# kostastril/Aiyagari-Replication

Hardware: AMD Instinct MI355X
Metric: Bellman evals/sec (Na·Na'·Nz, fp64) (higher is better)
Workload: dtype f64; 1 GPU; aiyagari_vfi_sweep Na=20000 Nz=7 rouwenhorst (BASELINE configs[1]); Na=20000, Nz=7, search=exhaustive over a' (exact bound-tree screen)

## Files before the change

### aiyagari-replication_amd/csrc/bellman.hpp

```cpp
#pragma once
#include <hip/hip_runtime.h>
#include <stddef.h>

#include "dispatch.hpp"

namespace aiy {

struct BellArgs {
    int N, Na, Nl;
    bool keep_incoming;
    bool labor;
    int np;
    int coarse;
    int CK;
    int variant;
    double r, w, beta, sigma;
    const double* v_old;
    const double* a;
    const double* s;
    const double* P;
    const double* L;
    const double* dis;
    const int* hint;
    int* mom;
    const int* perm;
    int perm_slots;
    int tw;
    double* EV;
    double2* T;
    float* T32;
    double* Dm;
    double* Dt;
    double* Dm8;
    double* Dm512;
    int nb, nb8, nb512;
    bool tree;
    double* best0;
    int* idx0;
    int* kf;
    bool kf_valid;
    int* partial;
    int* touched;
    unsigned long long* hitcount;
    long long* trace;
// ... 120 lines not shown
```

### aiyagari-replication_amd/csrc/bellman_kernels.hip

```cpp
#include <hip/hip_ext.h>

#include <algorithm>
#include <type_traits>

#include "aiy_common.hpp"
#include "bell_dev.hpp"
#include "bellman.hpp"

namespace aiy {

__device__ __forceinline__ BellArgs bell_cand(const BellArgs& A, int c) {
    BellArgs B = A;
    const size_t o = (size_t)c * A.N * A.Na;
    B.r = A.rv[c];
    B.w = A.wv[c];
    B.v_old += o;
    B.EV += o;
    if (B.Dt) B.Dt += o;
    if (B.Dm8) B.Dm8 += (size_t)c * A.N * A.nb8;
    if (B.Dm512) B.Dm512 += (size_t)c * A.N * A.nb512;
    B.kf += o * A.Nl;
    B.best0 += o;
    B.idx0 += o;
    if (B.hint) B.hint += o;
// ... 735 lines not shown
                    int dir = kb >= hk + wnh ? 1 : (kb <= hk - wnh ? -1 : 0);
                    if (usem && kb >= hm - mw && kb <= hm + mw)
                        dir = kb == hm + mw ? 1 : (kb == hm - mw ? -1 : 0);
                    if (dir != 0 && !(A.variant & kVarNoClimb)) {
                        int k = kb, step = 2;
                        for (;;) {
                            const int kn = min(max(k + dir * step, 0), kf - 1);
                            if (kn == k || !take(kn)) break;
                            k = kn;
                            step <<= 1;
                        }
                        for (int s2 = step >> 1; s2 >= 1; s2 >>= 1) {
                            const int c0 = idx[r] / Nl;
                            if (c0 + s2 < kf) take(c0 + s2);
                            if (c0 - s2 >= 0) take(c0 - s2);
                        }
                    }
                }
            }
        } else {
            best[r] = A.best0[t];
            idx[r] = A.idx0[t] == -2 ? -1 : A.idx0[t];
        }
    }
    int q_su[R];
    double kp_su[R];
#pragma unroll
    for (int r = 0; r < R; ++r) {
        q_su[r] = idx[r];
        kp_su[r] = a[idx[r] >= 0 ? idx[r] / Nl : 0];
    }
    unsigned nhits = nsu, nsup = 0, nwv = 0, nblk = 0, ngt = 0, nfine = 0, lane_pairs = 0;
    unsigned npath[2] = {0, 0};
    const long long t_start = (INS && A.trace) ? (long long)wall_clock64() : 0;
    long long cyc[4] = {0, 0, 0, 0}, c_mark = (INS && A.trace) ? (long long)__builtin_amdgcn_s_memtime() : 0;
    const long long c_mark0 = c_mark;
    auto stamp = [&](int ph) __attribute__((always_inline)) {
        if (INS && A.trace) {
            const long long now = (long long)__builtin_amdgcn_s_memtime();
            cyc[ph] += now - c_mark;
            c_mark = now;
        }
    };
    stamp(0);

    auto exchange = [&]() __attribute__((always_inline)) {
        if constexpr (W > 1) {
#pragma unroll
            for (int r = 0; r < R; ++r)
                s_cand[lw][r * 64 + lane] = make_double2(best[r], (double)idx[r]);
            __syncthreads();
            for (int v = 0; v < W; ++v)
#pragma unroll
                for (int r = 0; r < R; ++r) {
                    const double2 e = s_cand[v][r * 64 + lane];
                    if (v != wave && (int)e.y >= 0) lexi_take(e.x, (int)e.y, best[r], idx[r]);
                }
            __syncthreads();
        }
    };

    for (int l0 = 0; l0 < Nl; l0 += LB) {
        double coh[R][LB], B[R][LB], dis[LB];
        int kg = 0;
        int kfl = 0x7fffffff;
#pragma unroll
// ... 161 lines not shown
#pragma unroll
            for (int kk = 0; kk < 8; ++kk)
                vote |= (__any(GF ? pk[kk] && kk < nk : pk[kk]) ? 1u : 0u) << kk;
            if constexpr (!GF) vote &= (1u << (k1 - k0)) - 1u;
            if (!vote) return;
            stamp(2);
            while (vote) {
                const int kk = __builtin_ctz(vote);
                vote &= vote - 1;
                const int k = k0 + kk;
                const double2 tkk = s_cand[lw][k - sbase];
#pragma unroll
                for (int r = 0; r < R; ++r)
#pragma unroll
                    for (int q = 0; q < LB; ++q) {
                        const double c = coh[r][q] - tkk.x;
                        const int lin = (l0 + q) + Nl * k;
                        if (lin != idx[r] && c > 0 && (!GF || kk < nk) &&
                            (tkk.y - B[r][q]) * aiy_ipow(c, NP) >= kThr) {
                            ++nhits;
                            const double val =
                                bell_val<NP, LAB>(c, ev[k], A.sigma, dis[q]);
                            if (lexi_take(val, lin, best[r], idx[r])) {
#pragma unroll
                                for (int q2 = 0; q2 < LB; ++q2)
                                    if (B[r][q2] == B[r][q2])
                                        B[r][q2] = screen_B(best[r], idx[r], dis[q2], NP);
                            }
                        }
                    }
            }
            stamp(3);
        };
        auto load8 = [&](int sb, double& dm8, double& a8) __attribute__((always_inline)) {
            const int sub = (sb << 6) + lane;
            const bool oku = sub < A.nb8;
            dm8 = oku ? A.Dm8[(size_t)i * A.nb8 + sub] : -__builtin_inf();
            a8 = oku ? a[sub << 3] : 0.0;
        };
        auto stage = [&](int sbase, unsigned long long pass, double2 (&st)[8])
                         __attribute__((always_inline)) {
            if constexpr (LEAN) {
                unsigned bm = 0;
#pragma unroll
                for (int b = 0; b < 8; ++b) bm |= ((pass >> (8 * b)) & 0xffull) ? 1u << b : 0u;
                while (bm) {
                    const int b0 = __builtin_ctz(bm);
                    bm &= bm - 1;
                    const int b1 = bm ? __builtin_ctz(bm) : -1;
                    if (bm) bm &= bm - 1;
                    const int k0 = min(sbase + (b0 << 6) + lane, Na - 1);
                    const double2 v0 = make_double2(a[k0], Drow[k0]);
                    double2 v1 = make_double2(0.0, 0.0);
                    if (b1 >= 0) {
                        const int k1 = min(sbase + (b1 << 6) + lane, Na - 1);
                        v1 = make_double2(a[k1], Drow[k1]);
                    }
                    s_cand[lw][(b0 << 6) + lane] = v0;
                    if (b1 >= 0) s_cand[lw][(b1 << 6) + lane] = v1;
                }
            } else {
#pragma unroll
                for (int b = 0; b < 8; ++b)
                    if ((pass >> (8 * b)) & 0xffull) {
                        const int k = min(sbase + (b << 6) + lane, Na - 1);
                        st[b] = make_double2(a[k], Drow[k]);
                    }
            }
        };
        auto prep = [&](int sb, int bsel, int bstep, double dm8, double a8, double2 (&st)[8],
                        unsigned long long& gmo, bool subsplit = false)
                        __attribute__((always_inline)) -> unsigned long long {
            stamp(0);
            const int sbase = sb << 9;
            if constexpr (GRP) {
                constexpr int NG = 64 / GL, CH = LEAN ? 4 : 8;
                static_assert(NG % CH == 0, "whole chunks of groups");
                unsigned long long any = 0;
#pragma unroll
                for (int g0 = 0; g0 < NG; g0 += CH) {
                    double cx[CH], dd[CH], t[CH];
#pragma unroll
                    for (int u = 0; u < CH; ++u) {
                        cx[u] = readlane_d(gC, (g0 + u) * GL) - a8;
                        dd[u] = dm8 - readlane_d(gB, (g0 + u) * GL);
                    }
                    AIY_SCHED_BARRIER();
                    screen_t<NP, CH>(t, cx, dd);
#pragma unroll
                    for (int u = 0; u < CH; ++u) any |= __ballot(t[u] >= kThr);
                }
                if (INS && (A.hitcount || A.trace)) ngt += NG;
                const int nfe = min(64, (kg - sbase + 7) >> 3);
                unsigned long long pass = any & (nfe >= 64 ? ~0ull : (1ull << nfe) - 1ull);
                if (bstep > 1) {
                    const unsigned long long one = subsplit ? 0x01ull : 0xffull;
                    unsigned long long pat = one << (subsplit ? bsel : 8 * bsel);
                    for (int sh = subsplit ? bstep : 8 * bstep; sh < 64; sh <<= 1) pat |= pat << sh;
                    pass &= pat;
                }
                if (INS && (A.hitcount || A.trace)) nblk += __builtin_popcountll(pass);
                unsigned long long keep = 0, own = 0;
                for (unsigned long long m = pass; m; m &= m - 1) {
                    const int u = __builtin_ctzll(m);
                    const double dv = readlane_d(dm8, u), av = readlane_d(a8, u);
                    double cx[RL], dd[RL], t[RL];
#pragma unroll
                    for (int r = 0; r < R; ++r)
#pragma unroll
                        for (int q = 0; q < LB; ++q) {
                            cx[r * LB + q] = coh[r][q] - av;
                            dd[r * LB + q] = dv - B[r][q];
                        }
                    screen_t<NP, RL>(t, cx, dd);
                    bool p = false;
#pragma unroll
                    for (int m2 = 0; m2 < RL; ++m2) p = p || t[m2] >= kThr;
                    if (__any(p)) keep |= 1ull << u;
                    if constexpr (GF) own |= p ? 1ull << u : 0ull;
                }
                pass = keep;
                if constexpr (GF) gmo = keep ? group_or_u64(own) : 0ull;
                if (INS && A.trace && lane == 0) lane_pairs += __builtin_popcountll(pass);
                stage(sbase, pass, st);
                stamp(1);
// ... 5 lines not shown
            dm64 = fmax(dm64, dpp_d<0x104>(dm64));
            const int nblock = min(8, (kg - sbase + 63) >> 6);
            unsigned own = 0;
            for (int b = subsplit ? 0 : bsel; b < nblock; b += subsplit ? 1 : bstep) own |= 1u << b;
            if (INS && (A.hitcount || A.trace)) nblk += __builtin_popcount(own);
            const unsigned bpass = mask8(dm64, a8, 0, 8, nblock) & own;
            unsigned long long pass = 0;
            const bool deal = subsplit && bstep > 1;
            int ord = 0;
            for (unsigned bm = bpass; bm; bm &= bm - 1, ++ord) {
                if (deal && ord % bstep != bsel) continue;
                const int b = __builtin_ctz(bm);
                const int nsub = min(8, (kg - (sbase + (b << 6)) + 7) >> 3);
                if (INS && (A.hitcount || A.trace)) nblk += nsub;
                pass |= (unsigned long long)mask8(dm8, a8, 8 * b, 1, nsub, true) << (8 * b);
            }
            if constexpr (W > 1) {
                if (deal) {
                    s_pass[bsel] = pass;
                    __syncthreads();
                    unsigned long long all = 0;
                    for (int v = 0; v < bstep; ++v) all |= s_pass[v];
                    __syncthreads();
                    const unsigned long long pat = bstep == 2 ? 0x5555555555555555ull
                                                 : (bstep == 4 ? 0x1111111111111111ull
                                                               : 0x0101010101010101ull);
                    pass = all & (pat << bsel);
                }
            }
            stage(sbase, pass, st);
            stamp(1);
            return pass;
        };
        auto finish = [&](int sb, unsigned long long pass, const double2 (&st)[8],
                          unsigned long long gm) __attribute__((always_inline)) {
            const int sbase = sb << 9;
            if constexpr (!LEAN)
#pragma unroll
                for (int b = 0; b < 8; ++b)
                    if ((pass >> (8 * b)) & 0xffull) s_cand[lw][(b << 6) + lane] = st[b];
            __builtin_amdgcn_wave_barrier();
            __builtin_amdgcn_fence(__ATOMIC_RELEASE, "wavefront");
            stamp(1);
            double2 tkA[8], tkB[8];
            unsigned long long pm = pass;
            if constexpr (LEAN) {
                for (; pm; pm &= pm - 1) {
                    const int b0 = __builtin_ctzll(pm);
                    load_tk(b0, tkA);
                    fine(sbase, sbase + (b0 << 3), min(sbase + (b0 << 3) + 8, kg), tkA);
                }
            }
            if constexpr (GF) {
                pm = 0;
                const int hb = 63 - __builtin_clzll(pass);
                const bool ncl = FAST && sbase + (hb << 3) + 8 <= kfmin;
                auto next = [&](int& k0) __attribute__((always_inline)) {
                    const unsigned lo = (unsigned)gm, hi = (unsigned)(gm >> 32);
                    const unsigned tl = lo ? (unsigned)__builtin_ctz(lo) : ~0u;
                    const unsigned th = hi ? ((unsigned)__builtin_ctz(hi) | 32u) : ~0u;
                    const int b = (int)min(min(tl, th), (unsigned)hb);
                    gm &= gm - 1;
                    k0 = sbase + (b << 3);
                    return b;
                };
                int kA, kB;
                bool actA = gm != 0, actB;
                load_tk(next(kA), tkA);
                for (;;) {
// ... 5 lines not shown
                    actA = gm != 0;
                    const bool moreA = __any(actA);
                    if (moreA) load_tk(next(kA), tkA);
                    fine(sbase, kB, 0, tkB, actB, ncl);
                    if (!moreA) break;
                }
            }
            if (pm) load_tk(__builtin_ctzll(pm), tkA);
            while (pm) {
                const int b0 = __builtin_ctzll(pm);
                pm &= pm - 1;
                if (pm) load_tk(__builtin_ctzll(pm), tkB);
                fine(sbase, sbase + (b0 << 3), min(sbase + (b0 << 3) + 8, kg), tkA);
                if (!pm) break;
                const int b1 = __builtin_ctzll(pm);
                pm &= pm - 1;
                if (pm) load_tk(__builtin_ctzll(pm), tkA);
                fine(sbase, sbase + (b1 << 3), min(sbase + (b1 << 3) + 8, kg), tkB);
            }
            stamp(2);
            __builtin_amdgcn_wave_barrier();
        };

        const int nsb = (kg + 511) >> 9;
        int sfirst = -1;
        {
            int hk = -1;
#pragma unroll
            for (int r = 0; r < R; ++r)
                if (idx[r] >= 0) hk = idx[r] / Nl;
            const unsigned long long m = __ballot(hk >= 0);
            if (m) sfirst = min(readlane_i(hk, __builtin_ctzll(m)) >> 9, nsb - 1);
        }
        double2 st_cur[8], st_prev[8];
        if (sfirst >= 0) {
            if (INS) ++nsup;
            double d8, a8;
            load8(sfirst, d8, a8);
            unsigned long long gm1 = 0;
            const unsigned long long p = prep(sfirst, wave, W, d8, a8, st_cur, gm1,
                                              (A.variant & kVarDealBlocks) != 0);
            if (p) finish(sfirst, p, st_cur, gm1);
            exchange();
            set_B();
        }
        double dm0, a0;
        auto load512 = [&](int g) __attribute__((always_inline)) {
            const int sbl = g + lane;
            const bool oks = sbl < nsb;
            dm0 = oks ? A.Dm512[(size_t)i * A.nb512 + sbl] : -__builtin_inf();
            a0 = oks ? a[sbl << 9] : 0.0;
        };
        if (l0 == 0) {
            dm0 = dm0_pre;
            a0 = a0_pre;
        } else {
            load512(0);
        }
        double bmin, cmax;
        {
            if constexpr (GRP) {
                if (sfirst >= 0) set_G();
                bmin = wave_rest_fmin_d(gB);
                cmax = wave_rest_fmax_d(gC);
            } else {
                double bl = __builtin_nan(""), cl = -__builtin_inf();
#pragma unroll
                for (int r = 0; r < R; ++r)
#pragma unroll
                    for (int q = 0; q < LB; ++q) {
                        bl = fmin(bl, B[r][q]);
                        cl = fmax(cl, (okr[r] && l0 + q < Nl) ? coh[r][q] : -__builtin_inf());
                    }
                bmin = wave_fmin_d(bl);
                cmax = wave_fmax_d(cl);
            }
        }
        int g = 0;
        unsigned long long sm = 0;
        auto test512 = [&]() __attribute__((always_inline)) {
            if (INS) ++nwv;
            unsigned long long m =
                __ballot(lane < nsb - g && screen_wave<NP>(dm0, a0, bmin, cmax));
            static_assert(64 % W == 0, "superblock g + u belongs to wave u % W");
            if constexpr (W > 1) m &= (~0ull / ((1ull << W) - 1ull)) << wave;
            if (sfirst >= g && sfirst < g + 64) m &= ~(1ull << (sfirst - g));
            return m;
        };
        if (nsb > 0) sm = test512();
        auto next_sb = [&]() __attribute__((always_inline)) -> int {
            for (;;) {
                if (sm) {
                    const int u = __builtin_ctzll(sm);
                    sm &= sm - 1;
                    if (INS) ++nsup;
                    return g + u;
                }
                g += 64;
                if (g >= nsb) return -1;
                load512(g);
                sm = test512();
            }
        };
        int cur = nsb > 0 ? next_sb() : -1;
        double pd = 0.0, pa = 0.0;
        if (cur >= 0) load8(cur, pd, pa);
        unsigned long long pass_prev = 0, gm_cur = 0, gm_prev = 0;
        int sb_prev = -1;
        while (cur >= 0) {
            const double d8 = pd, a8 = pa;
            const int nxt = next_sb();
            if (nxt >= 0) load8(nxt, pd, pa);
            const unsigned long long pc = prep(cur, 0, 1, d8, a8, st_cur, gm_cur);
            if constexpr (LEAN) {
                if (pc) finish(cur, pc, st_cur, gm_cur);
                cur = nxt;
                continue;
            }
            if (pass_prev) finish(sb_prev, pass_prev, st_prev, gm_prev);
#pragma unroll
            for (int b = 0; b < 8; ++b) st_prev[b] = st_cur[b];
            pass_prev = pc;
            gm_prev = gm_cur;
            sb_prev = cur;
            cur = nxt;
        }
        if (pass_prev) finish(sb_prev, pass_prev, st_prev, gm_prev);
    }

    exchange();
    const long long c_end = (INS && A.trace) ? (long long)__builtin_amdgcn_s_memtime() : 0;

    bool okd = false;
    double dmax = 0.0;
#pragma unroll
    for (int r = 0; r < R; ++r) {
        if (!okr[r] || wave != 0) continue;
        const size_t t = (size_t)i * Na + jbase + r * 64 + lane;
        double b = best[r];
        int q = idx[r];
        const double vo = vo_pre[r];
        if (!feas[r] && LAB) {
            b = A.keep_incoming ? A.v_new[t] : vo;
        } else {
            if (q < 0) {
                q = 0;
                b = __builtin_nan("");
            }
            const int l = q % Nl, k = q / Nl;
            double kp = kp_su[r];
            if (__ballot(q != q_su[r]) != 0ull) kp = a[k];
            A.idx[t] = q;
            if (A.pk) A.pk[t] = kp;
            if (A.pc) A.pc[t] = cash<LAB>(x[r], y, LAB ? A.L[l] : 1.0) - kp;
            if (LAB && A.pl) A.pl[t] = A.L[l];
        }
        A.v_new[t] = b;
        if (mom && A.hint) {
            const int sh = (hk0[r] >= 0 && idx[r] >= 0) ? idx[r] / Nl - hk0[r] : 0;
            const int shc = max(-32767, min(32767, sh));
// ... 27 lines not shown
            for (int c = 0; c < 4; ++c) {
                unsigned sum = 0;
                for (int v = 0; v < W; ++v) sum += s_cnt[v][c];
                sums[c] = sum;
            }
        }
        if (W == 1 ? lane == 0 : threadIdx.x == 0) {
            long long* tr = A.trace + 16 * (size_t)item;
            tr[0] = t_start;
            tr[1] = (long long)wall_clock64();
            tr[2] = (long long)(unsigned)__builtin_amdgcn_s_getreg((20 << 0) | (0 << 6) | (3 << 11)) |
                    ((long long)(unsigned)__builtin_amdgcn_s_getreg((4 << 0) | (0 << 6) | (31 << 11))
                     << 32);
            for (int c = 0; c < 4; ++c) tr[3 + c] = sums[c];
            tr[7] = block_id;
            for (int c = 0; c < 4; ++c) tr[8 + c] = cyc[c];
            tr[12] = t_boot;
            tr[13] = c_mark0 - c_boot;
            tr[14] = (long long)__builtin_amdgcn_s_memtime() - c_end;
            tr[15] = pairs;
        }
    }
    if (INS && A.hitcount) {
        unsigned long long* hc = A.hitcount + 4 * (blockIdx.x % kDiffSlots);
        if (nhits) atomicAdd(hc, (unsigned long long)nhits);
        if (lane == 0) {
            const unsigned long long ns = 64ull * R * LB;
            atomicAdd(hc + 1, nwv * 64ull);
            atomicAdd(hc + 2, nblk * ns + ngt * 64ull);
            if (nfine) atomicAdd(hc + 3, nfine * ns);
#pragma unroll
            for (int q = 0; q < 2; ++q)
                if (npath[q]) atomicAdd(hc + kPathBase + q, (unsigned long long)npath[q]);
        }
    }
}

template <int NP, bool LAB, int R, int LB, int W, bool INS, int PK, int WM>
__global__ __launch_bounds__(64 * W * PK, 3) void bell_tree_kernel(BellArgs A0, int ntile) {
    __shared__ double2 s_cand[W * PK][512];
    __shared__ unsigned long long s_pass[W];
    const int lw = PK > 1 ? readfirst(threadIdx.x >> 6) : 0;
    bell_tree_item<NP, LAB, R, LB, W, INS, PK, false, WM>(A0, ntile, (int)blockIdx.x * PK + lw,
                                                          (int)gridDim.x * PK, s_cand, s_pass);
}

template <int NP, bool INS>
__global__ __launch_bounds__(128, 3) void bell_tree_hybrid_kernel(BellArgs A0, int ntile) {
    __shared__ double2 s_cand[2][512];
    __shared__ unsigned long long s_pass[2];
    const int b = (int)blockIdx.x;
    if (A0.perm[2 * b + 1] == -2) {
        bell_tree_item<NP, false, 1, 1, 2, INS, 1, true>(A0, ntile, 2 * b, 2 * (int)gridDim.x,
                                                        s_cand, s_pass);
    } else {
        const int lw = readfirst(threadIdx.x >> 6);
        bell_tree_item<NP, false, 1, 1, 1, INS, 2, true>(A0, ntile, 2 * b + lw,
                                                        2 * (int)gridDim.x, s_cand, s_pass);
    }
}

template <int NP, bool LAB, int LB>
__global__ void bell_merge_kernel(BellArgs A, int use_partial, int nlb, int nchunk) {
    int t = blockIdx.x * blockDim.x + threadIdx.x;
    bool ok = false;
    double d = 0.0;
// ... 382 lines not shown
```

### aiyagari-replication_amd/csrc/capi.cpp

```cpp
#include <hip/hip_runtime.h>

#include <algorithm>
#include <cmath>
#include <cstdarg>
#include <cstdlib>
#include <cstring>
#include <mutex>
#include <string>
#include <thread>
#include <vector>

#include "aiy_common.hpp"
#include "tree_perm.hpp"
#include "wide_batch.hpp"
#include "ws.hpp"

namespace aiy {

int wait_event(hipEvent_t ev) {
    for (int spin = 0;; ++spin) {
        const hipError_t e = hipEventQuery(ev);
        if (e == hipSuccess) return AIY_OK;
        if (e != hipErrorNotReady) {
            (void)hipGetLastError();
// ... 90 lines not shown
        ws->launches++;
    }
    ws->ev_used = 0;
    return AIY_OK;
}

bool tree_perm_eligible(const BellArgs& A);
int ws_tree_perm(aiy_ws* ws, const BellArgs& A, hipStream_t st);
static int bell_args(aiy_ws* ws, const BellCall& c, BellArgs& A, hipStream_t st) {
    if (!ws) return fail(AIY_BAD_ARG, "NULL workspace");
    if (!c.v_old || !c.a || !c.s || !c.P || !c.v_new || !c.idx)
        return fail(AIY_BAD_ARG, "NULL device pointer");
    if (c.labor && (!c.L || c.Nl < 1 || c.Nl > ws->Nl))
        return fail(AIY_BAD_ARG, "labour sweep needs labor_choice and 1 <= Nl <= workspace Nl");
    if (!(c.beta == c.beta) || !(c.r == c.r) || !(c.w == c.w) || !(c.sigma == c.sigma))
        return fail(AIY_NON_FINITE, "non-finite scalar argument");
    A = BellArgs{};
    A.N = (int)ws->N;
    A.Na = (int)ws->Na;
    A.Nl = c.labor ? (int)c.Nl : 1;
    A.labor = c.labor;
    A.keep_incoming = c.keep_incoming;
    A.np = is_int_ge(c.sigma, 2.0) && c.sigma <= 9.0 ? (int)c.sigma - 1 : 0;
    if (c.mode == 1 && A.np == 0)
        return fail(AIY_BAD_ARG, "screened sweep (mode 1) needs integer sigma in [2, 9]");
    A.coarse = ws->coarse;
    A.CK = ws->CK;
    const int var = ws->variant >= 0 ? ws->variant
                    : ws->Na <= 4096 ? (c.labor ? var_waves(2) | kVarDealBlocks : var_waves(1))
                    : (c.labor ? kVarXcdOrder | kVarDriftExtrap
                               : kVarXcdOrder | kVarPermCheapLast | var_pack(1) | kVarDriftExtrap |
                                     kVarHintAlone | kVarNoHintEval);
    A.variant = var;
    A.ev_mfma = bell_ev_mfma(A.N, ws->variant);
    A.tw = 0;
    if ((var & kVarNarrowTiles) && !c.labor && (var & kVarGeometryMask) == 0) {
        const int64_t tw = (ws->N * ws->Na + 3 * 1024 - 1) / (3 * 1024);
        A.tw = (int)std::max<int64_t>(16, std::min<int64_t>(64, tw));
        if (A.tw == 64) A.tw = 0;
    }
    A.r = c.r;
    A.w = c.w;
    A.beta = c.beta;
    A.sigma = c.sigma;
    A.v_old = c.v_old;
    A.a = c.a;
    A.s = c.s;
    A.P = c.P;
    A.L = c.labor ? c.L : nullptr;
    A.hint = c.hint;
    AIY_TRY(ws_ensure_bell(ws, bell_partial_slots(A)));
    A.dis = c.labor ? ws->dis : nullptr;
    A.EV = ws->EV;
    A.T = ws->T;
    A.tree = (var & kVarChunked) == 0;
    A.T32 = (A.tree || (var & kVarFp64Screen)) ? nullptr : ws->T32;
    A.Dm = A.tree ? nullptr : ws->Dm;
    A.Dm8 = A.tree ? ws->Dm8 : nullptr;
    A.Dt = A.tree ? ws->Dt : nullptr;
    A.Dm512 = A.tree ? ws->Dm512 : nullptr;
    A.nb = (int)((ws->Na + 63) / 64);
    A.nb8 = (int)((ws->Na + 7) / 8);
    A.nb512 = (int)((ws->Na + 511) / 512);
    A.best0 = ws->best0;
    A.idx0 = ws->idx0;
    A.mom = ws->mom;
// ... 362 lines not shown
        return AIY_OK;
    }
    if ((size_t)C * n > (size_t)INT32_MAX) return fail(AIY_BAD_SHAPE, "C*N*Na must fit int32");
    const int nb8 = (int)((ws->Na + 7) / 8), nb512 = (int)((ws->Na + 511) / 512);
    BatchBlocks& bb = ws->batch;
    if (bb.C != C) {
        bb = BatchBlocks{};
        AIY_TRY(bb.EV.ensure(C * n));
        AIY_TRY(bb.Dt.ensure(C * n));
        AIY_TRY(bb.Dm8.ensure((size_t)C * ws->N * nb8));
        AIY_TRY(bb.Dm512.ensure((size_t)C * ws->N * nb512));
        AIY_TRY(bb.best0.ensure(C * n));
        AIY_TRY(bb.idx0.ensure(C * n));
        AIY_TRY(bb.mom.ensure(C * n));
        AIY_HIP(hipMemset(bb.mom, 0, C * n * sizeof(int)));
        AIY_TRY(bb.kf.ensure(C * n));
        AIY_TRY(bb.stop.ensure((size_t)C));
        AIY_TRY(bb.slots.ensure((size_t)C * 2 * 2 * kDiffSlots));
        AIY_TRY(bb.rw.ensure(2 * (size_t)C));
        AIY_TRY(bb.hstop.ensure((size_t)C));
        AIY_TRY(bb.hslots.ensure((size_t)C * 2 * kDiffSlots));
        bb.C = C;
    }
    AIY_TRY(ws_ensure_bell(ws, 1));
    AIY_HIP(hipMemcpyAsync(bb.rw, r, C * sizeof(double), hipMemcpyHostToDevice, st));
    AIY_HIP(hipMemcpyAsync(bb.rw + C, w, C * sizeof(double), hipMemcpyHostToDevice, st));
    AIY_HIP(hipMemsetAsync(bb.stop, 0, C * sizeof(int), st));
    BellArgs A{};
    A.N = (int)ws->N; A.Na = (int)ws->Na; A.Nl = 1; A.labor = false; A.np = np;
    A.coarse = ws->coarse; A.CK = ws->CK;
    A.variant = ws->variant >= 0 ? ws->variant
                                   : (ws->Na <= 4096 ? 0 : kVarXcdOrder | kVarDriftExtrap);
    A.variant &= ~kVarGeometryMask;
    A.ev_mfma = bell_ev_mfma(A.N, ws->variant);
    A.beta = beta; A.sigma = sigma; A.a = a; A.s = s; A.P = P;
    A.EV = bb.EV; A.Dt = bb.Dt; A.Dm8 = bb.Dm8; A.Dm512 = bb.Dm512;
    A.nb = (int)((ws->Na + 63) / 64); A.nb8 = nb8; A.nb512 = nb512;
    A.tree = true; A.best0 = bb.best0; A.idx0 = bb.idx0; A.kf = bb.kf; A.mom = bb.mom;
    A.hitcount = ws->count_hits ? ws->hitcount : nullptr;
    A.idx = idx; A.pk = pk; A.pc = pc; A.diff = bb.slots;
    A.C = (int)C; A.rv = bb.rw; A.wv = bb.rw + C; A.stop = bb.stop;
    AIY_TRY(launch_bell_kf(A, st));
    ws->kf_ok = false;
    double* buf[2] = {v_a, v_b};
    int64_t g = 0;
    bool all_stopped = false;
    const int64_t m = std::max(ws->spec_max, 1);
    while (!all_stopped && g < max_iter) {
        const int64_t gend = std::min(max_iter, g + m);
        for (++g; g <= gend; ++g) {
            A.v_old = buf[(g - 1) & 1];
            A.v_new = buf[g & 1];
            A.parity = (int)(g & 1);
            A.hint = (g == 1 && !use_hint) ? nullptr : idx;
            if (A.ev_mfma) AIY_TRY(launch_bell_ev_mfma(A, st));
            AIY_TRY(launch_bell_table_batch(A, bb.slots, (int)g, tol, st));
            if (!A.hint) AIY_TRY(launch_bell_init(A, st));
            AIY_TRY(ws_timing_begin(ws, st));
            AIY_TRY(launch_bell_tree(A, st));
            AIY_TRY(ws_timing_end(ws, st));
        }
        --g;
        AIY_HIP(hipMemcpyAsync(bb.hstop, bb.stop, C * sizeof(int), hipMemcpyDeviceToHost, st));
        AIY_HIP(hipStreamSynchronize(st));
        all_stopped = true;
        for (int64_t c = 0; c < C; ++c) all_stopped = all_stopped && bb.hstop[c] != 0;
// ... 216 lines not shown
        *hits = c[0];
    }
    return AIY_OK;
}

int aiy_ws_counters(aiy_ws* ws, int64_t out[4]) {
    if (!ws || !out) return fail(AIY_BAD_ARG, "NULL workspace/out");
    std::vector<unsigned long long> h(4 * kDiffSlots, 0ull);
    if (ws->hitcount)
        AIY_HIP(hipMemcpy(h.data(), ws->hitcount, h.size() * sizeof(unsigned long long),
                          hipMemcpyDeviceToHost));
    for (int q = 0; q < 4; ++q) {
        unsigned long long t = 0;
        for (int sl = 0; sl < kDiffSlots; ++sl) t += h[4 * sl + q];
        out[q] = (int64_t)t;
    }
    return AIY_OK;
}

int aiy_ws_screen_paths(aiy_ws* ws, int64_t out[2]) {
    if (!ws || !out) return fail(AIY_BAD_ARG, "NULL workspace/out");
    std::vector<unsigned long long> h(kHitcountLen, 0ull);
    if (ws->hitcount)
        AIY_HIP(hipMemcpy(h.data(), ws->hitcount, h.size() * sizeof(unsigned long long),
                          hipMemcpyDeviceToHost));
    for (int q = 0; q < 2; ++q) {
        unsigned long long t = 0;
        for (int sl = 0; sl < kDiffSlots; ++sl) t += h[kPathBase + 4 * sl + q];
        out[q] = (int64_t)t;
    }
    return AIY_OK;
}

int aiy_ws_trace(aiy_ws* ws, int64_t* out, int64_t cap, int64_t* n) {
    if (!ws || !out || !n) return fail(AIY_BAD_ARG, "NULL argument");
    *n = 0;
    if (!ws->trace) return AIY_OK;
    int64_t m = std::min(cap, ws_trace_units(ws));
    AIY_HIP(hipMemcpy(out, ws->trace, 16 * (size_t)m * sizeof(int64_t), hipMemcpyDeviceToHost));
    *n = m;
    return AIY_OK;
}

int aiy_ws_invalidate(aiy_ws* ws) {
    if (!ws) return fail(AIY_BAD_ARG, "NULL workspace");
    ws->kf_ok = false;
    ws->dis_ok = false;
    return AIY_OK;
}

int aiy_ws_set_variant(aiy_ws* ws, int variant) {
    if (!ws) return fail(AIY_BAD_ARG, "NULL workspace");
    if (variant < -1 || variant >= (1 << 30)) return fail(AIY_BAD_ARG, "variant in [-1, 2^30)");
    ws->variant = variant;
    return AIY_OK;
}

int aiy_ws_set_wide(aiy_ws* ws, int max_na, int splits, int waves, int states) {
    if (!ws) return fail(AIY_BAD_ARG, "NULL workspace");
    if (max_na < -1 || splits < 0 || splits > kWideMaxSplits ||
        (waves != 0 && waves != 4 && waves != 8 && waves != 16) ||
        (states != 0 && states != 8 && states != 16 && states != 32 && states != 64))
        return fail(AIY_BAD_ARG, "max_na >= -1, splits in [0, %d], waves in {0, 4, 8, 16}, "
                    "states in {0, 8, 16, 32, 64}", kWideMaxSplits);
    ws->wide_max = max_na;
    ws->wide_S = splits;
    ws->wide_NW = waves;
    ws->wide_SB = states;
    return AIY_OK;
}

int aiy_ws_set_cu_exclusive(aiy_ws* ws, int on) {
    if (!ws) return fail(AIY_BAD_ARG, "NULL workspace");
    ws->cu_exclusive = on != 0;
    return AIY_OK;
}

int aiy_ws_set_speculation(aiy_ws* ws, int max_batch) {
    if (!ws) return fail(AIY_BAD_ARG, "NULL workspace");
    if (max_batch < 0 || max_batch > 256) return fail(AIY_BAD_ARG, "max_batch in [0, 256]");
    if (max_batch != ws->spec_max) ws->spec = SpecRings{};
    ws->spec_max = max_batch;
    return AIY_OK;
}

int aiy_ws_set_search(aiy_ws* ws, int coarse_stride, int k_chunk) {
    if (!ws) return fail(AIY_BAD_ARG, "NULL workspace");
// ... 131 lines not shown
```

### aiyagari-replication_amd/csrc/ws.hpp

```cpp
#pragma once
#include <hip/hip_runtime.h>

#include "aiy_common.hpp"
#include "bellman.hpp"
#include "devbuf.hpp"

namespace aiy {
using u64 = unsigned long long;
struct SpecRings {
    size_t n = 0;
    int m = 0;
    DevBuf<double> v;
    DevBuf<int> idx;
    DevBuf<double> pol;
    DevBuf<u64> diff;
    PinnedBuf<u64> hdiff;
    Events ev;
};
struct SlotRings {
    size_t n = 0;
    int m = 0;
    DevBuf<double> ring;
    DevBuf<u64> slots;
    PinnedBuf<u64> hslots;
// ... 23 lines not shown
};
struct LaborBatchBlocks {
    int64_t C = 0;
    DevBuf<int> kf;
    DevBuf<int> stop;
    DevBuf<u64> slots;
    DevBuf<double> rw;
    PinnedBuf<int> hstop;
    PinnedBuf<u64> hslots;
};
struct TransitionBlocks {
    DevBuf<double> rw;
    DevBuf<int> res;
    PinnedBuf<double> hrw;
    PinnedBuf<int> hres;
    int ensure(size_t C, size_t T) {
        AIY_TRY(rw.ensure(C * (2 * T + 1)));
        AIY_TRY(res.ensure(2 * C));
        AIY_TRY(hrw.ensure(C * (2 * T + 1)));
        return hres.ensure(2 * C);
    }
};
}

struct aiy_ws {
    template <class T>
    using Dev = aiy::DevBuf<T>;
    using u64 = aiy::u64;
    int64_t N = 0, Na = 0, Nl = 1;
    int dev = 0;
    int coarse = 512;
    int CK = 1024;
    int variant = -1;
    Dev<double> EV;
    Dev<double2> T;
    Dev<float> T32;
    Dev<double> Dm, Dm8, Dt, Dm512, best0;
    Dev<int> idx0;
    Dev<int> mom;
    Dev<int> touched;
    Dev<double> dis;
    Dev<int> kf;
    bool kf_ok = false;
    double kf_r = 0, kf_w = 0;
    const void* kf_a = nullptr;
    const void* kf_s = nullptr;
    const void* kf_L = nullptr;
    int64_t kf_Nl = 0;
    bool kf_lab = false;
    Dev<int> tree_perm;
    int perm_slots = 0;
    long long perm_key = 0;
    Dev<int> kf_last;
    bool dis_ok = false;
    const void* dis_L = nullptr;
    int64_t dis_Nl = 0;
    double dis_psi = 0, dis_eta = 0;
    int wide_max = -1, wide_S = 0, wide_NW = 0, wide_SB = 0;
    bool cu_exclusive = false;
    int sim_par = -1;
    Dev<double> sim_kbuf;
    Dev<u64> wdiff;
    int wcur = 0;
    Dev<unsigned> wcnt;
    Dev<u64> wpart;
    bool last_wide = false;
// ... 91 lines not shown
```

### aiyagari-replication_amd/vfi.py

```python
from __future__ import annotations

import ctypes as C

import numpy as np

from ._capi import check, d, i64, ip, lib, ptr, stream_handle, vp


def _f(a):
    return np.asfortranarray(a, dtype=np.float64)


def vfi_sweep(v_old, a_grid, s, P, r, w, beta, sigma):
    v_old = _f(v_old)
    N, Na = v_old.shape
    a_grid, s = np.ascontiguousarray(a_grid, np.float64), np.ascontiguousarray(s, np.float64)
    P = _f(P)
    v_new = np.empty((N, Na), order="F"); pk = np.empty((N, Na), order="F")
    pc = np.empty((N, Na), order="F"); idx = np.empty((N, Na), np.int32, order="F")
    check(lib().aiy_vfi_sweep(ptr(v_old), ptr(a_grid), ptr(s), ptr(P), i64(N), i64(Na), d(r),
                              d(w), d(beta), d(sigma), ptr(v_new), ptr(pk), ptr(pc), ptr(idx)))
    return v_new, pk, pc, idx


# ... 41 lines not shown
    def trace(self):
        items = self.N * ((self.Na + 7) // 8)
        cap = max(self.N * ((self.Na + 15) // 16), (items + 7) // 8 * 8 * 16)
        out = np.zeros((cap, 16), np.int64)
        n = C.c_int64(0)
        check(lib().aiy_ws_trace(self._h, out.ctypes.data_as(C.c_void_p), i64(cap), C.byref(n)))
        out = out[:n.value]
        return out[out[:, 1] > 0]

    def trace_wide(self):
        items = self.N * ((self.Na + 7) // 8)
        cap = (items + 7) // 8 * 8 * 16 * 4
        out = np.zeros((cap, 16), np.int64)
        n = C.c_int64(0)
        check(lib().aiy_ws_trace(self._h, out.ctypes.data_as(C.c_void_p), i64(cap), C.byref(n)))
        out = out[:n.value - n.value % 4].reshape(-1, 64)
        return out[out[:, 1] > 0]

    def timing(self):
        ms, n, hits = C.c_double(0), C.c_int64(0), C.c_int64(0)
        check(lib().aiy_ws_timing(self._h, C.byref(ms), C.byref(n), C.byref(hits)))
        return ms.value, n.value, hits.value

    def counters(self):
        out = (C.c_int64 * 4)()
        check(lib().aiy_ws_counters(self._h, out))
        return tuple(int(x) for x in out)

    def screen_paths(self):
        out = (C.c_int64 * 2)()
        check(lib().aiy_ws_screen_paths(self._h, out))
        return tuple(int(x) for x in out)

    def invalidate(self):
        check(lib().aiy_ws_invalidate(self._h))

    def set_egm_batch(self, min_candidates: int = -1):
        check(lib().aiy_ws_set_egm_batch(self._h, ip(min_candidates)))

    def egm_batch_counts(self):
        a, b = C.c_int64(0), C.c_int64(0)
        check(lib().aiy_ws_egm_batch_counts(self._h, C.byref(a), C.byref(b)))
        return a.value, b.value

    def set_labor_batch(self, min_candidates: int = 0):
        check(lib().aiy_ws_set_labor_batch(self._h, ip(min_candidates)))

    def labor_batch_counts(self):
        a, b = C.c_int64(0), C.c_int64(0)
        check(lib().aiy_ws_labor_batch_counts(self._h, C.byref(a), C.byref(b)))
        return a.value, b.value

    def set_dist_batch(self, min_candidates: int = -1):
        check(lib().aiy_ws_set_dist_batch(self._h, ip(min_candidates)))

    def dist_batch_counts(self):
        a, b = C.c_int64(0), C.c_int64(0)
        check(lib().aiy_ws_dist_batch_counts(self._h, C.byref(a), C.byref(b)))
        return a.value, b.value

    def set_variant(self, variant: int):
        check(lib().aiy_ws_set_variant(self._h, ip(variant)))

    def set_speculation(self, max_batch: int):
        check(lib().aiy_ws_set_speculation(self._h, ip(max_batch)))

    def set_wide(self, max_na: int = -1, splits: int = 0, waves: int = 0, states: int = 0):
        check(lib().aiy_ws_set_wide(self._h, ip(max_na), ip(splits), ip(waves), ip(states)))

    def set_cu_exclusive(self, on: bool = True):
        check(lib().aiy_ws_set_cu_exclusive(self._h, ip(int(bool(on)))))

    def set_sim(self, mode: int = -1):
        check(lib().aiy_ws_set_sim(self._h, ip(int(mode))))

    def set_search(self, coarse_stride=0, k_chunk=1024):
        check(lib().aiy_ws_set_search(self._h, ip(coarse_stride), ip(k_chunk)))

    def vfi_sweep(self, v_old, a_grid, s, P, r, w, beta, sigma, v_new, idx, policy_k=None,
                  policy_c=None, hint=None, mode=0, diff=None, stream=None):
        check(lib().aiy_vfi_sweep_dev(self._h, ptr(v_old), ptr(a_grid), ptr(s), ptr(P), d(r),
                                      d(w), d(beta), d(sigma), ptr(hint), ip(mode), ptr(v_new),
                                      ptr(idx), ptr(policy_k), ptr(policy_c), ptr(diff),
                                      stream_handle(stream)))

    def vfi_sweeps(self, v_a, v_b, a_grid, s, P, r, w, beta, sigma, nsweeps, idx,
                   policy_k=None, policy_c=None, hint=None, mode=0, diff=None, stream=None):
        check(lib().aiy_vfi_sweeps_dev(self._h, ptr(v_a), ptr(v_b), ptr(a_grid), ptr(s), ptr(P),
                                       d(r), d(w), d(beta), d(sigma), ptr(hint), i64(nsweeps),
                                       ip(mode), ptr(idx), ptr(policy_k), ptr(policy_c),
                                       ptr(diff), stream_handle(stream)))

    def vfi_solve(self, v_a, v_b, a_grid, s, P, r, w, beta, sigma, tol, max_iter, idx,
                  policy_k=None, policy_c=None, mode=0, stream=None):
        it, which = C.c_int64(0), C.c_int(0)
# ... 104 lines not shown
```

### include/aiyagari_hip.h

```cpp
#ifndef AIYAGARI_HIP_H
#define AIYAGARI_HIP_H
#include <stdint.h>
#ifdef __cplusplus
extern "C" {
#endif

typedef enum {
    AIY_OK = 0,
    AIY_BAD_SHAPE = 1,
    AIY_NON_FINITE = 2,
    AIY_HIP_ERROR = 3,
    AIY_RCCL_ERROR = 4,
    AIY_NO_DEVICE = 5,
    AIY_BAD_ARG = 6,
    AIY_FIND_EMPTY = 7,
    AIY_NO_MEMORY = 8
} aiy_status;

const char* aiy_last_error(void);
int aiy_version(void);
int aiy_device_count(void);


int aiy_release_all(void);
// ... 129 lines not shown
int ks_shocks(int64_t T, int64_t population, const double* uniforms, const double* params,
              double* zi_shock, double* epsi_shock);

int ks_simulate_capital(const double* k_opt, const double* k_grid, const double* K_grid,
                        int64_t nk, int64_t nK, const double* zi_shock,
                        const double* epsi_shock, int64_t T, int64_t population,
                        double* k_population, double* K_ts);

int ks_simulate_hist(const double* k_opt, const double* k_grid, const double* K_grid, int64_t nk,
                     int64_t nK, const double* x_grid, int64_t nx, const double* params,
                     const double* zi_shock, int64_t T, int64_t M, double* lam, double* K_ts,
                     int64_t* slow_periods);
int ks_simulate_hist_multi(int64_t C, const double* k_opt, const double* k_grid,
                           const double* K_grid, int64_t nk, int64_t nK, const double* x_grid,
                           int64_t nx, const double* params, const int32_t* policy_of_path,
                           const double* zi_shock, int64_t T, int64_t M, double* lam,
                           double* K_ts, int64_t* slow_periods);

typedef struct aiy_ws aiy_ws;
int aiy_ws_create(int64_t N, int64_t Na, int64_t Nl, aiy_ws** ws);
int aiy_ws_destroy(aiy_ws* ws);
int aiy_ws_set_timing(aiy_ws* ws, int enable);
int aiy_ws_timing(aiy_ws* ws, double* total_ms, int64_t* launches, int64_t* hits);
int aiy_ws_counters(aiy_ws* ws, int64_t out[4]);
int aiy_ws_screen_paths(aiy_ws* ws, int64_t out[2]);
int aiy_ws_trace(aiy_ws* ws, int64_t* out, int64_t cap, int64_t* n);
int aiy_ws_invalidate(aiy_ws* ws);
int aiy_ws_set_search(aiy_ws* ws, int coarse_stride, int k_chunk);
int aiy_ws_set_speculation(aiy_ws* ws, int max_batch);
int aiy_ws_set_wide(aiy_ws* ws, int max_na, int splits, int waves, int states);
int aiy_ws_set_cu_exclusive(aiy_ws* ws, int on);
int aiy_ws_set_sim(aiy_ws* ws, int mode);
int aiy_ws_set_variant(aiy_ws* ws, int variant);

int aiy_vfi_sweep_dev(aiy_ws* ws, const double* v_old, const double* a_grid, const double* s,
                      const double* P, double r, double w, double beta, double sigma,
                      const int32_t* hint, int mode, double* v_new, int32_t* idx,
                      double* policy_k, double* policy_c, double* diff, void* stream);
int aiy_vfi_sweeps_dev(aiy_ws* ws, double* v_a, double* v_b, const double* a_grid,
                       const double* s, const double* P, double r, double w, double beta,
                       double sigma, const int32_t* hint, int64_t nsweeps, int mode, int32_t* idx,
                       double* policy_k, double* policy_c, double* diff, void* stream);
int aiy_vfi_solve_dev(aiy_ws* ws, double* v_a, double* v_b, const double* a_grid,
                      const double* s, const double* P, double r, double w, double beta,
                      double sigma, double tol, int64_t max_iter, int mode, int32_t* idx,
                      double* policy_k, double* policy_c, int64_t* iters, int* out_new,
                      void* stream);
int aiy_vfi_solve_batch_dev(aiy_ws* ws, int64_t C, const double* r, const double* w,
                            double* v_a, double* v_b, const double* a_grid, const double* s,
                            const double* P, double beta, double sigma, double tol,
                            int64_t max_iter, int use_hint, int32_t* idx, double* policy_k,
                            double* policy_c, int64_t* iters, int32_t* which, void* stream);
int aiy_labor_vfi_sweep_dev(aiy_ws* ws, const double* v_old, const double* a_grid,
                            const double* s, const double* P, const double* labor_choice,
                            double r, double w, double beta, double sigma, double psi,
                            double eta, const int32_t* hint, double* v_new, int32_t* lin,
                            double* policy_k, double* policy_l, double* policy_c, double* diff,
                            void* stream);
int aiy_labor_vfi_sweeps_dev(aiy_ws* ws, double* v_a, double* v_b, const double* a_grid,
                             const double* s, const double* P, const double* labor_choice,
                             double r, double w, double beta, double sigma, double psi,
                             double eta, const int32_t* hint, int64_t nsweeps, int32_t* lin,
                             double* policy_k, double* policy_l, double* policy_c, double* diff,
                             void* stream);
int aiy_labor_vfi_solve_batch_dev(aiy_ws* ws, int64_t C, const double* r, const double* w,
                                  double* v_a, double* v_b, const double* a_grid,
// ... 151 lines not shown
```

Measured before the change: 105900 billion evals/s.

## Center first evaluated superblock window on hinted policy span in tree screen

Instead of evaluating the first 512-wide superblock aligned at the hint's block, the tree kernel now evaluates a 512-wide window centered on the midpoint of the wave's hinted policy indices, aligned to 64. This aims to raise the initial best values sooner so that later bound screens prune more superblocks. The two straddled superblocks are excluded from the rescan only when a group test over the parts outside the window shows no candidates. It is enabled by default for large non-labor grids with the default variant, and adds counters plus an API toggle. The cost is an extra Dm8 load and an extra group test per row, with some risk of an edge-case correctness error in the exclusion logic.

Result: no change. 105300 billion evals/s (-0.6%).

```diff
diff --git a/aiyagari-replication_amd/csrc/bellman.hpp b/aiyagari-replication_amd/csrc/bellman.hpp
--- a/aiyagari-replication_amd/csrc/bellman.hpp
+++ b/aiyagari-replication_amd/csrc/bellman.hpp
@@ -10,6 +10,7 @@
     int N, Na, Nl;
     bool keep_incoming;
     bool labor;
+    bool first_window;
     int np;
     int coarse;
     int CK;
diff --git a/aiyagari-replication_amd/csrc/bellman_kernels.hip b/aiyagari-replication_amd/csrc/bellman_kernels.hip
--- a/aiyagari-replication_amd/csrc/bellman_kernels.hip
+++ b/aiyagari-replication_amd/csrc/bellman_kernels.hip
@@ -791,6 +791,7 @@
     }
     unsigned nhits = nsu, nsup = 0, nwv = 0, nblk = 0, ngt = 0, nfine = 0, lane_pairs = 0;
     unsigned npath[2] = {0, 0};
+    unsigned nwin = 0, nfb = 0;
     const long long t_start = (INS && A.trace) ? (long long)wall_clock64() : 0;
     long long cyc[4] = {0, 0, 0, 0}, c_mark = (INS && A.trace) ? (long long)__builtin_amdgcn_s_memtime() : 0;
     const long long c_mark0 = c_mark;
@@ -1018,8 +1019,8 @@
             }
             stamp(3);
         };
-        auto load8 = [&](int sb, double& dm8, double& a8) __attribute__((always_inline)) {
-            const int sub = (sb << 6) + lane;
+        auto load8 = [&](int sbase, double& dm8, double& a8) __attribute__((always_inline)) {
+            const int sub = (sbase >> 3) + lane;
             const bool oku = sub < A.nb8;
             dm8 = oku ? A.Dm8[(size_t)i * A.nb8 + sub] : -__builtin_inf();
             a8 = oku ? a[sub << 3] : 0.0;
@@ -1054,29 +1055,33 @@
                     }
             }
         };
-        auto prep = [&](int sb, int bsel, int bstep, double dm8, double a8, double2 (&st)[8],
+        auto group_test = [&](double dm8, double a8) __attribute__((always_inline))
+                              -> unsigned long long {
+            constexpr int NG = 64 / GL, CH = LEAN ? 4 : 8;
+            static_assert(NG % CH == 0, "whole chunks of groups");
+            unsigned long long any = 0;
+#pragma unroll
+            for (int g0 = 0; g0 < NG; g0 += CH) {
+                double cx[CH], dd[CH], t[CH];
+#pragma unroll
+                for (int u = 0; u < CH; ++u) {
+                    cx[u] = readlane_d(gC, (g0 + u) * GL) - a8;
+                    dd[u] = dm8 - readlane_d(gB, (g0 + u) * GL);
+                }
+                AIY_SCHED_BARRIER();
+                screen_t<NP, CH>(t, cx, dd);
+#pragma unroll
+                for (int u = 0; u < CH; ++u) any |= __ballot(t[u] >= kThr);
+            }
+            if (INS && (A.hitcount || A.trace)) ngt += NG;
+            return any;
+        };
+        auto prep = [&](int sbase, int bsel, int bstep, double dm8, double a8, double2 (&st)[8],
                         unsigned long long& gmo, bool subsplit = false)
                         __attribute__((always_inline)) -> unsigned long long {
             stamp(0);
-            const int sbase = sb << 9;
             if constexpr (GRP) {
-                constexpr int NG = 64 / GL, CH = LEAN ? 4 : 8;
-                static_assert(NG % CH == 0, "whole chunks of groups");
-                unsigned long long any = 0;
-#pragma unroll
-                for (int g0 = 0; g0 < NG; g0 += CH) {
-                    double cx[CH], dd[CH], t[CH];
-#pragma unroll
-                    for (int u = 0; u < CH; ++u) {
-                        cx[u] = readlane_d(gC, (g0 + u) * GL) - a8;
-                        dd[u] = dm8 - readlane_d(gB, (g0 + u) * GL);
-                    }
-                    AIY_SCHED_BARRIER();
-                    screen_t<NP, CH>(t, cx, dd);
-#pragma unroll
-                    for (int u = 0; u < CH; ++u) any |= __ballot(t[u] >= kThr);
-                }
-                if (INS && (A.hitcount || A.trace)) ngt += NG;
+                const unsigned long long any = group_test(dm8, a8);
                 const int nfe = min(64, (kg - sbase + 7) >> 3);
                 unsigned long long pass = any & (nfe >= 64 ? ~0ull : (1ull << nfe) - 1ull);
                 if (bstep > 1) {
@@ -1148,9 +1153,8 @@
             stamp(1);
             return pass;
         };
-        auto finish = [&](int sb, unsigned long long pass, const double2 (&st)[8],
+        auto finish = [&](int sbase, unsigned long long pass, const double2 (&st)[8],
                           unsigned long long gm) __attribute__((always_inline)) {
-            const int sbase = sb << 9;
             if constexpr (!LEAN)
 #pragma unroll
                 for (int b = 0; b < 8; ++b)
@@ -1222,15 +1226,37 @@
             const unsigned long long m = __ballot(hk >= 0);
             if (m) sfirst = min(readlane_i(hk, __builtin_ctzll(m)) >> 9, nsb - 1);
         }
+        constexpr bool FW = GF && !(NP == 1 && WM != 1);
+        int wbase = -1, nlo = 0;
+        double cd8 = -__builtin_inf(), ca8 = 0.0;
+        if constexpr (FW) {
+            if (A.first_window && A.hint && sfirst >= 0) {
+                const unsigned long long m = __ballot(idx[0] >= 0);
+                const int klo = readlane_i(idx[0], __builtin_ctzll(m));
+                const int khi = readlane_i(idx[0], 63 - __builtin_clzll(m));
+                const int c = (int)(((long long)klo + khi) >> 1);
+                wbase = max(0, min((c - 256) & ~63, (nsb << 9) - 512));
+                nlo = (wbase & 511) >> 3;
+                if (nlo) {
+                    const int cblk =
+                        lane < nlo ? ((wbase >> 9) << 6) + lane : (wbase >> 3) + 64 + lane - nlo;
+                    const bool okc = (cblk << 3) < kg;
+                    cd8 = okc ? A.Dm8[(size_t)i * A.nb8 + cblk] : -__builtin_inf();
+                    ca8 = okc ? a[cblk << 3] : 0.0;
+                }
+                if (INS) ++nwin;
+            }
+        }
         double2 st_cur[8], st_prev[8];
         if (sfirst >= 0) {
             if (INS) ++nsup;
+            const int sb1 = (FW && wbase >= 0) ? wbase : sfirst << 9;
             double d8, a8;
-            load8(sfirst, d8, a8);
+            load8(sb1, d8, a8);
             unsigned long long gm1 = 0;
-            const unsigned long long p = prep(sfirst, wave, W, d8, a8, st_cur, gm1,
+            const unsigned long long p = prep(sb1, wave, W, d8, a8, st_cur, gm1,
                                               (A.variant & kVarDealBlocks) != 0);
-            if (p) finish(sfirst, p, st_cur, gm1);
+            if (p) finish(sb1, p, st_cur, gm1);
             exchange();
             set_B();
         }
@@ -1266,6 +1292,19 @@
                 cmax = wave_fmax_d(cl);
             }
         }
+        int ex0 = sfirst, ex1 = -1;
+        if constexpr (FW) {
+            if (wbase >= 0) {
+                ex0 = wbase >> 9;
+                if (nlo) {
+                    const unsigned long long cm = group_test(cd8, ca8);
+                    ex1 = ex0 + 1;
+                    if (cm & ((1ull << nlo) - 1ull)) ex0 = -1;
+                    if (cm >> nlo) ex1 = -1;
+                    if (INS) nfb += (ex0 < 0 ? 1u : 0u) + (ex1 < 0 ? 1u : 0u);
+                }
+            }
+        }
         int g = 0;
         unsigned long long sm = 0;
         auto test512 = [&]() __attribute__((always_inline)) {
@@ -1274,7 +1313,9 @@
                 __ballot(lane < nsb - g && screen_wave<NP>(dm0, a0, bmin, cmax));
             static_assert(64 % W == 0, "superblock g + u belongs to wave u % W");
             if constexpr (W > 1) m &= (~0ull / ((1ull << W) - 1ull)) << wave;
-            if (sfirst >= g && sfirst < g + 64) m &= ~(1ull << (sfirst - g));
+            if (ex0 >= g && ex0 < g + 64) m &= ~(1ull << (ex0 - g));
+            if constexpr (FW)
+                if (ex1 >= g && ex1 < g + 64) m &= ~(1ull << (ex1 - g));
             return m;
         };
         if (nsb > 0) sm = test512();
@@ -1294,20 +1335,20 @@
         };
         int cur = nsb > 0 ? next_sb() : -1;
         double pd = 0.0, pa = 0.0;
-        if (cur >= 0) load8(cur, pd, pa);
+        if (cur >= 0) load8(cur << 9, pd, pa);
         unsigned long long pass_prev = 0, gm_cur = 0, gm_prev = 0;
         int sb_prev = -1;
         while (cur >= 0) {
             const double d8 = pd, a8 = pa;
             const int nxt = next_sb();
-            if (nxt >= 0) load8(nxt, pd, pa);
-            const unsigned long long pc = prep(cur, 0, 1, d8, a8, st_cur, gm_cur);
+            if (nxt >= 0) load8(nxt << 9, pd, pa);
+            const unsigned long long pc = prep(cur << 9, 0, 1, d8, a8, st_cur, gm_cur);
             if constexpr (LEAN) {
-                if (pc) finish(cur, pc, st_cur, gm_cur);
+                if (pc) finish(cur << 9, pc, st_cur, gm_cur);
                 cur = nxt;
                 continue;
             }
-            if (pass_prev) finish(sb_prev, pass_prev, st_prev, gm_prev);
+            if (pass_prev) finish(sb_prev << 9, pass_prev, st_prev, gm_prev);
 #pragma unroll
             for (int b = 0; b < 8; ++b) st_prev[b] = st_cur[b];
             pass_prev = pc;
@@ -1315,7 +1356,7 @@
             sb_prev = cur;
             cur = nxt;
         }
-        if (pass_prev) finish(sb_prev, pass_prev, st_prev, gm_prev);
+        if (pass_prev) finish(sb_prev << 9, pass_prev, st_prev, gm_prev);
     }
 
     exchange();
@@ -1409,6 +1450,8 @@
 #pragma unroll
             for (int q = 0; q < 2; ++q)
                 if (npath[q]) atomicAdd(hc + kPathBase + q, (unsigned long long)npath[q]);
+            if (nwin) atomicAdd(hc + kPathBase + 2, (unsigned long long)nwin);
+            if (nfb) atomicAdd(hc + kPathBase + 3, (unsigned long long)nfb);
         }
     }
 }
diff --git a/aiyagari-replication_amd/csrc/capi.cpp b/aiyagari-replication_amd/csrc/capi.cpp
--- a/aiyagari-replication_amd/csrc/capi.cpp
+++ b/aiyagari-replication_amd/csrc/capi.cpp
@@ -146,6 +146,8 @@
                                : kVarXcdOrder | kVarPermCheapLast | var_pack(1) | kVarDriftExtrap |
                                      kVarHintAlone | kVarNoHintEval);
     A.variant = var;
+    A.first_window = ws->first_window >= 0 ? ws->first_window != 0
+                                           : (ws->variant < 0 && ws->Na > 4096 && !c.labor);
     A.ev_mfma = bell_ev_mfma(A.N, ws->variant);
     A.tw = 0;
     if ((var & kVarNarrowTiles) && !c.labor && (var & kVarGeometryMask) == 0) {
@@ -574,6 +576,7 @@
     A.variant = ws->variant >= 0 ? ws->variant
                                    : (ws->Na <= 4096 ? 0 : kVarXcdOrder | kVarDriftExtrap);
     A.variant &= ~kVarGeometryMask;
+    A.first_window = ws->first_window == 1;
     A.ev_mfma = bell_ev_mfma(A.N, ws->variant);
     A.beta = beta; A.sigma = sigma; A.a = a; A.s = s; A.P = P;
     A.EV = bb.EV; A.Dt = bb.Dt; A.Dm8 = bb.Dm8; A.Dm512 = bb.Dm512;
@@ -856,6 +859,20 @@
     return AIY_OK;
 }
 
+int aiy_ws_first_window(aiy_ws* ws, int64_t out[2]) {
+    if (!ws || !out) return fail(AIY_BAD_ARG, "NULL workspace/out");
+    std::vector<unsigned long long> h(kHitcountLen, 0ull);
+    if (ws->hitcount)
+        AIY_HIP(hipMemcpy(h.data(), ws->hitcount, h.size() * sizeof(unsigned long long),
+                          hipMemcpyDeviceToHost));
+    for (int q = 0; q < 2; ++q) {
+        unsigned long long t = 0;
+        for (int sl = 0; sl < kDiffSlots; ++sl) t += h[kPathBase + 4 * sl + 2 + q];
+        out[q] = (int64_t)t;
+    }
+    return AIY_OK;
+}
+
 int aiy_ws_trace(aiy_ws* ws, int64_t* out, int64_t cap, int64_t* n) {
     if (!ws || !out || !n) return fail(AIY_BAD_ARG, "NULL argument");
     *n = 0;
@@ -877,6 +894,13 @@
     if (!ws) return fail(AIY_BAD_ARG, "NULL workspace");
     if (variant < -1 || variant >= (1 << 30)) return fail(AIY_BAD_ARG, "variant in [-1, 2^30)");
     ws->variant = variant;
+    return AIY_OK;
+}
+
+int aiy_ws_set_first_window(aiy_ws* ws, int mode) {
+    if (!ws) return fail(AIY_BAD_ARG, "NULL workspace");
+    if (mode < -1 || mode > 1) return fail(AIY_BAD_ARG, "first-window mode in {-1, 0, 1}");
+    ws->first_window = mode;
     return AIY_OK;
 }
 
diff --git a/aiyagari-replication_amd/csrc/ws.hpp b/aiyagari-replication_amd/csrc/ws.hpp
--- a/aiyagari-replication_amd/csrc/ws.hpp
+++ b/aiyagari-replication_amd/csrc/ws.hpp
@@ -79,6 +79,7 @@
     int coarse = 512;
     int CK = 1024;
     int variant = -1;
+    int first_window = -1;
     Dev<double> EV;
     Dev<double2> T;
     Dev<float> T32;
diff --git a/aiyagari-replication_amd/vfi.py b/aiyagari-replication_amd/vfi.py
--- a/aiyagari-replication_amd/vfi.py
+++ b/aiyagari-replication_amd/vfi.py
@@ -97,6 +97,11 @@
         check(lib().aiy_ws_screen_paths(self._h, out))
         return tuple(int(x) for x in out)
 
+    def first_window(self):
+        out = (C.c_int64 * 2)()
+        check(lib().aiy_ws_first_window(self._h, out))
+        return tuple(int(x) for x in out)
+
     def invalidate(self):
         check(lib().aiy_ws_invalidate(self._h))
 
@@ -126,6 +131,9 @@
 
     def set_variant(self, variant: int):
         check(lib().aiy_ws_set_variant(self._h, ip(variant)))
+
+    def set_first_window(self, mode: int = -1):
+        check(lib().aiy_ws_set_first_window(self._h, ip(mode)))
 
     def set_speculation(self, max_batch: int):
         check(lib().aiy_ws_set_speculation(self._h, ip(max_batch)))
diff --git a/include/aiyagari_hip.h b/include/aiyagari_hip.h
--- a/include/aiyagari_hip.h
+++ b/include/aiyagari_hip.h
@@ -185,6 +185,8 @@
 int aiy_ws_set_cu_exclusive(aiy_ws* ws, int on);
 int aiy_ws_set_sim(aiy_ws* ws, int mode);
 int aiy_ws_set_variant(aiy_ws* ws, int variant);
+int aiy_ws_set_first_window(aiy_ws* ws, int mode);
+int aiy_ws_first_window(aiy_ws* ws, int64_t out[2]);
 
 int aiy_vfi_sweep_dev(aiy_ws* ws, const double* v_old, const double* a_grid, const double* s,
                       const double* P, double r, double w, double beta, double sigma,
```
